# archinetai/audio-diffusion-pytorch

Measured on NVIDIA H100. Metric: audio-seconds/sec (2ch, 2^18 len) VSampler 50-step, higher is better.
Workload: dtype bf16

## Files before the change

### audio_diffusion_pytorch_b200/csrc/conv_gemm.cu

```cuda
#include "common.cuh"
#include "ptx.cuh"

namespace adp {

int g_debug[8] = {0, 0, 0, 0, 0, 0, 0, 0};

constexpr int kBM = 128;
constexpr int kMaxStages = 8;
constexpr int kMaxGroups = 8;
constexpr int kConsumers = 256;
constexpr int kGemmThreads = kConsumers + 32;
constexpr int kSmemPerSM = 228 * 1024;
constexpr int kSmemPerBlock = 227 * 1024;

struct Gemm2Params {
  __nv_bfloat16* out;
  const __nv_bfloat16* residual;
  const float* bias;
  const float* gate;
  double* stats;
  int B, T, tiles_per_batch, c_in, ldo;
  int n_pad, n_valid;
  int ntaps, tap_off0, up_factor;
  int groups, group_size, group_shift;
  int out_fp32, ld_gate;
  int n_tiles_n, total_tiles, tiles_per_cta;
  int a_rows;
  int kc;
  int k_stages;
  int n_stages;
  int a_sub_bytes, w_sub_bytes, stage_bytes, max_taps;
  int early_w;
  const double* gn_stats;
  const float* gn_gamma;
  const float* gn_beta;
  float gn_eps;
  int gn_groups;
};

struct TileInfo {
  int b, t0, n0, phase, ch0, ntaps, min_off;
};

__device__ __forceinline__ TileInfo tile_info(const Gemm2Params& p, int tile, int BN) {
  TileInfo ti;
  const int m_tile = tile / p.n_tiles_n;
  const int n_tile = tile - m_tile * p.n_tiles_n;
  ti.b = m_tile / p.tiles_per_batch;
  ti.t0 = (m_tile - ti.b * p.tiles_per_batch) * kBM;
  ti.n0 = n_tile * BN;
  ti.phase = ti.n0 / p.n_pad;
  ti.ch0 = ti.n0 - ti.phase * p.n_pad;
  if (p.up_factor > 1) {
    if (ti.phase == 0) { ti.ntaps = 2; ti.min_off = -1; }
    else if (ti.phase == p.up_factor - 1) { ti.ntaps = 2; ti.min_off = 0; }
    else { ti.ntaps = 1; ti.min_off = 0; }
  } else {
    ti.ntaps = p.ntaps;
    ti.min_off = p.tap_off0;
  }
  return ti;
}

__device__ __forceinline__ float silu_tanh(float z) {
  float t;
  asm("tanh.approx.f32 %0, %1;" : "=f"(t) : "f"(0.5f * z));
  const float hz = 0.5f * z;
  return fmaf(hz, t, hz);
}

struct WarpStats {
  int cur_g = -1;
  float s = 0.f, q = 0.f;
  __device__ __forceinline__ void flush(float (*slots)[8], int w, int lane) {
    const float ws = warp_sum(s), wq = warp_sum(q);
    if (lane == 0 && cur_g >= 0) { slots[2 * cur_g][w] += ws; slots[2 * cur_g + 1][w] += wq; }
    s = 0.f; q = 0.f;
  }
  __device__ __forceinline__ void add(float v, int g, float (*slots)[8], int w, int lane) {
    if (g != cur_g) { flush(slots, w, lane); cur_g = g; }
    s += v; q += v * v;
  }
};

struct NarrowStats {
  int ch0 = -1;
  float s[4] = {0.f, 0.f, 0.f, 0.f}, q[4] = {0.f, 0.f, 0.f, 0.f};
  __device__ __forceinline__ void add(int k, float v) { s[k] += v; q[k] += v * v; }
  __device__ __forceinline__ void flush(float (*slots)[8], int w, int lane, int shift, int groups) {
    if (ch0 >= 0) {
#pragma unroll
      for (int k = 0; k < 4; ++k) {
        float a = s[k], b = q[k];
#pragma unroll
        for (int o = 4; o < 32; o <<= 1) {
          a += __shfl_xor_sync(0xffffffffu, a, o);
          b += __shfl_xor_sync(0xffffffffu, b, o);
        }
        if (shift == 2) {
          a += __shfl_xor_sync(0xffffffffu, a, 1);
          b += __shfl_xor_sync(0xffffffffu, b, 1);
        }
        const int col = shift == 0 ? ch0 + 2 * lane + k : ch0 + 8 * k + 2 * (lane & 3);
        const int g = col >> shift;
        if (lane < 4 && (shift != 2 || !(lane & 1)) && (shift != 0 || k < 2) && g < groups) {
          slots[2 * g][w] += a;
          slots[2 * g + 1][w] += b;
        }
        s[k] = 0.f; q[k] = 0.f;
      }
    }
    ch0 = -1;
  }
};

template <int BN, int SW, bool XF, bool NARROW>
__global__ void __launch_bounds__(kGemmThreads, BN <= 32 ? 3 : (BN <= 64 ? 2 : 1))
conv_gemm2_kernel(const __grid_constant__ CUtensorMap tmA, const __grid_constant__ CUtensorMap tmW,
                  const Gemm2Params p) {
  static_assert(!NARROW || (BN <= 64 && !XF), "narrow statistics registers: BN <= 64 without XF");
  constexpr int BK = SW / 2;
  constexpr int NACC = BN / 2;
  constexpr uint32_t kWTapBytes = BN * SW;
  extern __shared__ uint8_t smem_raw[];
  __shared__ uint64_t full_bar[kMaxStages], empty_bar[kMaxStages];
  __shared__ float s_part[2 * kMaxGroups][8];
  __shared__ __align__(16) float s_coef[XF ? 2 * 1024 : 4];

  pdl_launch_dependents();
  const int warp = warp_id_uniform();
  const int lane = threadIdx.x & 31;
  const uint32_t raw = smem_u32(smem_raw);
  uint8_t* ring = smem_raw + ((1024u - (raw & 1023u)) & 1023u);

  const int tile_begin = blockIdx.x * p.tiles_per_cta;
  int tile_end = tile_begin + p.tiles_per_cta;
  if (tile_end > p.total_tiles) tile_end = p.total_tiles;

  if (threadIdx.x < 2 * kMaxGroups * 8) (&s_part[0][0])[threadIdx.x] = 0.f;
  if (warp == 8 && lane == 0) {
    for (int s = 0; s < p.n_stages; ++s) { mbar_init(&full_bar[s], 1); mbar_init(&empty_bar[s], 8); }
    fence_mbar_init();
    tma_prefetch_desc(&tmA);
    tma_prefetch_desc(&tmW);
  }
  __syncthreads();
  if (warp == 8) {
    const uint32_t a_bytes = static_cast<uint32_t>(p.a_rows) * SW;
    const int total_it = (tile_end - tile_begin) * p.k_stages;
    int early = 0;
    if (p.early_w) {
      early = total_it < p.n_stages ? total_it : p.n_stages;
      if (elect_one()) {
        int tile = tile_begin, ks = 0;
        for (int it = 0; it < early; ++it) {
          const TileInfo ti = tile_info(p, tile, BN);
          uint8_t* st = ring + it * p.stage_bytes;
          mbar_arrive_expect_tx(&full_bar[it], static_cast<uint32_t>(p.kc) * (a_bytes + ti.ntaps * kWTapBytes));
          for (int c = 0; c < p.kc; ++c) {
            const int k0 = (ks * p.kc + c) * BK;
            uint8_t* wdst = st + p.kc * p.a_sub_bytes + c * p.max_taps * p.w_sub_bytes;
            for (int tap = 0; tap < ti.ntaps; ++tap)
              tma_load_2d(wdst + tap * p.w_sub_bytes, &tmW, &full_bar[it], tap * p.c_in + k0, ti.n0);
          }
          if (++ks == p.k_stages) { ks = 0; ++tile; }
        }
      }
      __syncwarp();
    }
    pdl_wait();
    int s = 0, it = 0;
    uint32_t ph = 0;
    for (int tile = tile_begin; tile < tile_end; ++tile) {
      const TileInfo ti = tile_info(p, tile, BN);
      const uint32_t tx = static_cast<uint32_t>(p.kc) * (a_bytes + ti.ntaps * kWTapBytes);
      for (int ks = 0; ks < p.k_stages; ++ks, ++it) {
        const bool armed = it < early;
        if (!armed) mbar_wait(&empty_bar[s], ph ^ 1);
        uint8_t* st = ring + s * p.stage_bytes;
        if (elect_one()) {
          if (!armed) mbar_arrive_expect_tx(&full_bar[s], tx);
          for (int c = 0; c < p.kc; ++c) {
            const int k0 = (ks * p.kc + c) * BK;
            tma_load_3d(st + c * p.a_sub_bytes, &tmA, &full_bar[s], k0, ti.t0 + ti.min_off, ti.b);
            if (armed) continue;
            uint8_t* wdst = st + p.kc * p.a_sub_bytes + c * p.max_taps * p.w_sub_bytes;
            for (int tap = 0; tap < ti.ntaps; ++tap)
              tma_load_2d(wdst + tap * p.w_sub_bytes, &tmW, &full_bar[s], tap * p.c_in + k0, ti.n0);
          }
        }
        __syncwarp();
        if (++s == p.n_stages) { s = 0; ph ^= 1; }
      }
    }
    return;
  }

  pdl_wait();
  const int tid = threadIdx.x;
  const int wg = tid >> 7;
  const int r0 = wg * 64 + (warp & 3) * 16 + (lane >> 2);
  const int cq = 2 * (lane & 3);
  const bool do_stats = p.stats != nullptr;
  const bool narrow = NARROW && p.group_shift >= 0 && p.group_shift < 3;
  WarpStats acc_st;
  NarrowStats nar_st;
  int cur_b = -1, coef_b = -1;

  auto publish_stats = [&](int b_done) {
    acc_st.flush(s_part, warp, lane);
    acc_st.cur_g = -1;
    if (narrow) nar_st.flush(s_part, warp, lane, p.group_shift, p.groups);
    named_bar_sync(1, kConsumers);
    if (tid < 2 * p.groups) {
      float tot = 0.f;
#pragma unroll
      for (int w = 0; w < 8; ++w) { tot += s_part[tid][w]; s_part[tid][w] = 0.f; }
      if (tot != 0.f) atomicAdd(p.stats + static_cast<size_t>(b_done) * 2 * p.groups + tid, static_cast<double>(tot));
    }
    named_bar_sync(1, kConsumers);
  };

  const uint64_t desc0 = gmma_desc_kmajor<SW>(smem_u32(ring));
  const uint32_t stage_u = static_cast<uint32_t>(p.stage_bytes) >> 4;
  const uint32_t a_sub_u = static_cast<uint32_t>(p.a_sub_bytes) >> 4;
  const uint32_t w_sub_u = static_cast<uint32_t>(p.w_sub_bytes) >> 4;
  const uint32_t w_base_u = static_cast<uint32_t>(p.kc) * a_sub_u;
  const uint32_t wg_row_u = static_cast<uint32_t>(wg * 64 * SW) >> 4;
  int s = 0;
  uint32_t ph = 0;
  for (int tile = tile_begin; tile < tile_end; ++tile) {
    const TileInfo ti = tile_info(p, tile, BN);
    if constexpr (XF) {
      if (ti.b != coef_b) {
        named_bar_sync(1, kConsumers);
        const int gsz = p.c_in / p.gn_groups;
        const double inv_n = 1.0 / (static_cast<double>(gsz) * p.T);
        for (int ch = tid; ch < p.c_in; ch += kConsumers) {
          const int g = ch / gsz;
          const double mean = p.gn_stats[(static_cast<size_t>(ti.b) * p.gn_groups + g) * 2] * inv_n;
          const float var = fmaxf(static_cast<float>(
              p.gn_stats[(static_cast<size_t>(ti.b) * p.gn_groups + g) * 2 + 1] * inv_n - mean * mean), 0.f);
          const float ga = __ldg(p.gn_gamma + ch) * rsqrtf(var + p.gn_eps);
          s_coef[2 * ch] = ga;
          s_coef[2 * ch + 1] = __ldg(p.gn_beta + ch) - static_cast<float>(mean) * ga;
        }
        named_bar_sync(1, kConsumers);
        coef_b = ti.b;
      }
    }
    float acc[NACC];
    uint32_t accumulate = 0;
    int prev_s = -1;
    for (int ks = 0; ks < p.k_stages; ++ks) {
      mbar_wait(&full_bar[s], ph);
      if constexpr (XF) {
        constexpr int CPR = SW / 16;
        constexpr int CPT = CPR / 2 > 0 ? CPR / 2 : 1;
        uint8_t* st = ring + s * p.stage_bytes;
        for (int c = 0; c < p.kc; ++c) {
          uint8_t* sub = st + c * p.a_sub_bytes;
          const float* cf = s_coef + (ks * p.kc + c) * BK * 2;
          for (int rr = tid >> 1; rr < p.a_rows; rr += kConsumers / 2) {
            const int t = ti.t0 + ti.min_off + rr;
            if (t < 0 || t >= p.T) continue;
            const uint32_t row_off = static_cast<uint32_t>(rr) * SW;
            const int swz = (row_off >> 7) & (CPR - 1);
#pragma unroll
            for (int q = 0; q < CPT; ++q) {
              const int pc = (CPR >= 2) ? (tid & 1) * CPT + q : 0;
              if (CPR < 2 && (tid & 1)) continue;
              const int lc = pc ^ swz;
              uint4* ptr = reinterpret_cast<uint4*>(sub + row_off + pc * 16);
              const uint4 u = *ptr;
              const float4* c4 = reinterpret_cast<const float4*>(cf + lc * 16);
              const float4 k0 = c4[0], k1 = c4[1], k2 = c4[2], k3 = c4[3];
              const float2 f0 = unpack_bf16(u.x), f1 = unpack_bf16(u.y);
              const float2 f2 = unpack_bf16(u.z), f3 = unpack_bf16(u.w);
              uint4 o;
              o.x = pack_bf16(silu_tanh(f0.x * k0.x + k0.y), silu_tanh(f0.y * k0.z + k0.w));
              o.y = pack_bf16(silu_tanh(f1.x * k1.x + k1.y), silu_tanh(f1.y * k1.z + k1.w));
              o.z = pack_bf16(silu_tanh(f2.x * k2.x + k2.y), silu_tanh(f2.y * k2.z + k2.w));
              o.w = pack_bf16(silu_tanh(f3.x * k3.x + k3.y), silu_tanh(f3.y * k3.z + k3.w));
              *ptr = o;
            }
          }
        }
        fence_proxy_async_smem();
        named_bar_sync(1, kConsumers);
      }
      wgmma_fence();
      const uint64_t sdesc = desc0 + static_cast<uint64_t>(s * stage_u);
      for (int c = 0; c < p.kc; ++c) {
        const uint64_t adesc = sdesc + c * a_sub_u + wg_row_u;
        const uint64_t wdesc = sdesc + w_base_u + c * p.max_taps * w_sub_u;
        for (int tap = 0; tap < ti.ntaps; ++tap) {
#pragma unroll
          for (int kk = 0; kk < BK / 16; ++kk) {
            Wgmma<BN>::template ss<0, 0>(acc, adesc + ((tap * SW + kk * 32) >> 4),
                                         wdesc + tap * w_sub_u + ((kk * 32) >> 4), accumulate);
            accumulate = 1;
          }
        }
      }
      wgmma_commit();
      wgmma_wait<1>();
      if (prev_s >= 0) {
        __syncwarp();
        if (lane == 0) mbar_arrive(&empty_bar[prev_s]);
      }
      prev_s = s;
      if (++s == p.n_stages) { s = 0; ph ^= 1; }
    }
    wgmma_wait<0>();
    acc_fence(acc);
    __syncwarp();
    if (lane == 0) mbar_arrive(&empty_bar[prev_s]);

    if (do_stats && ti.b != cur_b) {
      if (cur_b >= 0) publish_stats(cur_b);
      cur_b = ti.b;
    }
    if (narrow && ti.ch0 != nar_st.ch0) {
      nar_st.flush(s_part, warp, lane, p.group_shift, p.groups);
      nar_st.ch0 = ti.ch0;
    }
    const int t_lo = ti.t0 + r0, t_hi = t_lo + 8;
    const bool ok_lo = t_lo < p.T, ok_hi = t_hi < p.T;
    const size_t col_off = static_cast<size_t>(ti.phase) * p.n_valid;
    const size_t off_lo = (static_cast<size_t>(ti.b) * p.T + (ok_lo ? t_lo : 0)) * p.ldo + col_off;
    const size_t off_hi = (static_cast<size_t>(ti.b) * p.T + (ok_hi ? t_hi : 0)) * p.ldo + col_off;
    const float* gate_row = p.gate ? p.gate + static_cast<size_t>(ti.b) * p.ld_gate : nullptr;
#pragma unroll
    for (int jb = 0; jb < BN / 8; ++jb) {
      if (ti.ch0 + jb * 8 >= p.n_valid) break;
      const int ch = ti.ch0 + jb * 8 + cq;
      const float2 bb = p.bias ? make_float2(__ldg(p.bias + ch), __ldg(p.bias + ch + 1)) : make_float2(0.f, 0.f);
      const float2 gg = gate_row ? make_float2(__ldg(gate_row + ch), __ldg(gate_row + ch + 1)) : make_float2(1.f, 1.f);
      float v[4];
      v[0] = (acc[4 * jb + 0] + bb.x) * gg.x; v[1] = (acc[4 * jb + 1] + bb.y) * gg.y;
      v[2] = (acc[4 * jb + 2] + bb.x) * gg.x; v[3] = (acc[4 * jb + 3] + bb.y) * gg.y;
      if (p.out_fp32) {
        float* o = reinterpret_cast<float*>(p.out);
        if (ok_lo) *reinterpret_cast<float2*>(o + off_lo + ch) = make_float2(v[0], v[1]);
        if (ok_hi) *reinterpret_cast<float2*>(o + off_hi + ch) = make_float2(v[2], v[3]);
        continue;
      }
      if (p.residual) {
        if (ok_lo) {
          const float2 r = unpack_bf16(__ldg(reinterpret_cast<const unsigned int*>(p.residual + off_lo + ch)));
          v[0] += r.x; v[1] += r.y;
        }
        if (ok_hi) {
          const float2 r = unpack_bf16(__ldg(reinterpret_cast<const unsigned int*>(p.residual + off_hi + ch)));
          v[2] += r.x; v[3] += r.y;
        }
      }
      const uint32_t o_lo = pack_bf16(v[0], v[1]), o_hi = pack_bf16(v[2], v[3]);
      if (ok_lo) *reinterpret_cast<uint32_t*>(p.out + off_lo + ch) = o_lo;
      if (ok_hi) *reinterpret_cast<uint32_t*>(p.out + off_hi + ch) = o_hi;
      if (do_stats) {
        const float2 q_lo = ok_lo ? unpack_bf16(o_lo) : make_float2(0.f, 0.f);
        const float2 q_hi = ok_hi ? unpack_bf16(o_hi) : make_float2(0.f, 0.f);
        if (p.group_shift >= 3) {
          const int g = (ti.ch0 + jb * 8) >> p.group_shift;
          acc_st.add(q_lo.x, g, s_part, warp, lane); acc_st.add(q_lo.y, g, s_part, warp, lane);
          acc_st.add(q_hi.x, g, s_part, warp, lane); acc_st.add(q_hi.y, g, s_part, warp, lane);
        } else if (narrow) {
          if (p.group_shift == 0) {
            nar_st.add(0, q_lo.x); nar_st.add(0, q_hi.x);
            nar_st.add(1, q_lo.y); nar_st.add(1, q_hi.y);
          } else if (jb < 4) {
            nar_st.add(jb, q_lo.x); nar_st.add(jb, q_lo.y);
            nar_st.add(jb, q_hi.x); nar_st.add(jb, q_hi.y);
          }
        } else {
          float cs[2] = {q_lo.x + q_hi.x, q_lo.y + q_hi.y};
          float cs2[2] = {q_lo.x * q_lo.x + q_hi.x * q_hi.x, q_lo.y * q_lo.y + q_hi.y * q_hi.y};
#pragma unroll
          for (int e = 0; e < 2; ++e)
#pragma unroll
            for (int o = 4; o < 32; o <<= 1) {
              cs[e] += __shfl_xor_sync(0xffffffffu, cs[e], o);
              cs2[e] += __shfl_xor_sync(0xffffffffu, cs2[e], o);
            }
#pragma unroll
          for (int i = 0; i < 8; ++i) {
            const float v = __shfl_sync(0xffffffffu, cs[i & 1], i >> 1);
            const float v2 = __shfl_sync(0xffffffffu, cs2[i & 1], i >> 1);
            const int g = (ti.ch0 + jb * 8 + i) / p.group_size;
            if (lane == 0) { s_part[2 * g][warp] += v; s_part[2 * g + 1][warp] += v2; }
          }
        }
      }
    }
  }
  if (do_stats && cur_b >= 0) publish_stats(cur_b);
}

template <int BN, int SW, bool XF, bool NARROW>
static int launch_gemm2(const adp_conv_gemm_args& a, cudaStream_t stream) {
  constexpr int BK = SW / 2;
  auto kernel = conv_gemm2_kernel<BN, SW, XF, NARROW>;
  const int tiles_per_batch = (a.T + kBM - 1) / kBM;
  const bool up = a.up_factor > 1;
  const int max_taps = up ? 2 : a.ntaps;
  const int span = up ? 1 : a.ntaps - 1;
  const int a_rows = kBM + span;
  const int k_chunks = a.c_in / BK;

  Gemm2Params p;
  p.a_sub_bytes = (a_rows * SW + 1023) / 1024 * 1024;
  p.w_sub_bytes = (BN * SW + 1023) / 1024 * 1024;
  p.max_taps = max_taps;
  const int chunk_bytes = p.a_sub_bytes + max_taps * p.w_sub_bytes;

  const int w_iters = k_chunks * max_taps;
  int occ = 1;
  if (BN <= 64 && w_iters <= 8) occ = 3;
  else if (BN <= 128 && w_iters <= 12) occ = 2;
  if (XF && occ > (BN <= 64 ? 2 : 1)) occ = BN <= 64 ? 2 : 1;
  if (g_debug[3] > 0) occ = g_debug[3];
  static int static_smem = -1;
  if (static_smem < 0) {
    cudaFuncAttributes fa;
    ADP_CUDA(cudaFuncGetAttributes(&fa, kernel));
    static_smem = static_cast<int>(fa.sharedSizeBytes);
  }
  auto budget_of = [&](int o) {
    int per_cta = kSmemPerSM / o - 1024;
    if (per_cta > kSmemPerBlock) per_cta = kSmemPerBlock;
    return per_cta - static_smem - 1024;
  };
  while (occ > 1 && budget_of(occ) < 2 * chunk_bytes) --occ;
  const int budget = budget_of(occ);
  int kc = 1;
  while (kc * 2 <= 4 && k_chunks % (kc * 2) == 0 && kc * max_taps * (BK / 16) < 8 &&
         2 * (kc * 2) * chunk_bytes <= budget)
    kc *= 2;
  if (g_debug[5] > 0 && k_chunks % g_debug[5] == 0) kc = g_debug[5];
  p.kc = kc;
  p.k_stages = k_chunks / kc;
  p.stage_bytes = kc * chunk_bytes;
  int n_stages = budget / p.stage_bytes;
  if (n_stages > kMaxStages) n_stages = kMaxStages;
  if (n_stages < 2)
    return set_error("adp_conv_gemm: stage of %d bytes does not fit (BN=%d)", p.stage_bytes, BN);
  p.n_stages = n_stages;
  const size_t smem = static_cast<size_t>(n_stages) * p.stage_bytes + 1024;

  CUtensorMap tmA, tmW;
  {
    const uint64_t dims[3] = {(uint64_t)a.c_in, (uint64_t)a.T, (uint64_t)a.B};
    const uint64_t strides[2] = {(uint64_t)a.lda * 2, (uint64_t)a.T * a.lda * 2};
    const uint32_t box[3] = {(uint32_t)BK, (uint32_t)a_rows, 1};
    if (int e = make_tmap_bf16(&tmA, a.a, 3, dims, strides, box, SW)) return e;
  }
  {
    const uint64_t dims[2] = {(uint64_t)a.k_total, (uint64_t)a.phases * a.n_pad};
    const uint64_t strides[1] = {(uint64_t)a.k_total * 2};
    const uint32_t box[2] = {(uint32_t)BK, (uint32_t)BN};
    if (int e = make_tmap_bf16(&tmW, a.w, 2, dims, strides, box, SW)) return e;
  }

  static SmemAttrCache smem_cache;
  ADP_CUDA(ensure_dyn_smem(kernel, smem, smem_cache));
  int occ_hw = 1;
  if (cudaOccupancyMaxActiveBlocksPerMultiprocessor(&occ_hw, kernel, kGemmThreads, smem) != cudaSuccess ||
      occ_hw < 1)
    occ_hw = 1;
  if (occ > occ_hw) occ = occ_hw;

  p.out = static_cast<__nv_bfloat16*>(a.out);
  p.residual = static_cast<const __nv_bfloat16*>(a.residual);
  p.bias = a.bias;
  p.gate = a.gate;
  p.stats = a.stats;
  p.B = a.B;
  p.T = a.T;
  p.tiles_per_batch = tiles_per_batch;
  p.c_in = a.c_in;
  p.ldo = a.ldo;
  p.n_pad = a.n_pad;
  p.n_valid = a.n_valid;
  p.ntaps = a.ntaps;
  p.tap_off0 = a.tap_off[0];
  p.up_factor = a.up_factor;
  p.groups = a.stats ? a.groups : 0;
  p.group_size = a.stats ? a.n_valid / a.groups : 1;
  p.group_shift = -1;
  for (int sft = 0; sft < 16; ++sft)
    if ((1 << sft) == p.group_size) p.group_shift = sft;
  p.out_fp32 = a.out_fp32;
  p.ld_gate = a.ld_gate > 0 ? a.ld_gate : a.n_valid;
  p.n_tiles_n = a.phases * a.n_pad / BN;
  p.total_tiles = a.B * tiles_per_batch * p.n_tiles_n;
  p.a_rows = a_rows;
  p.early_w = g_debug[2];
  p.gn_stats = a.gn_stats;
  p.gn_gamma = a.gn_gamma;
  p.gn_beta = a.gn_beta;
  p.gn_eps = a.gn_eps;
  p.gn_groups = a.gn_groups > 0 ? a.gn_groups : 1;

  const int slots = occ * num_sms();
  int grid = p.total_tiles < slots ? p.total_tiles : slots;
  p.tiles_per_cta = (p.total_tiles + grid - 1) / grid;
  grid = (p.total_tiles + p.tiles_per_cta - 1) / p.tiles_per_cta;
  ADP_CUDA(launch_k(kernel, dim3(grid), dim3(kGemmThreads), smem, stream, tmA, tmW, p));
  ADP_LAUNCH_CHECK();
  return 0;
}

template <int SW>
static int dispatch_bn2(const adp_conv_gemm_args& a, int bn, cudaStream_t s) {
  if (a.gn_stats) {
    switch (bn) {
      case 16: return launch_gemm2<16, SW, true, false>(a, s);
      case 32: return launch_gemm2<32, SW, true, false>(a, s);
      case 64: return launch_gemm2<64, SW, true, false>(a, s);
      case 128: return launch_gemm2<128, SW, true, false>(a, s);
      case 256: return launch_gemm2<256, SW, true, false>(a, s);
    }
  }
  const int group_size = a.stats ? a.n_valid / a.groups : 0;
  const bool narrow = group_size == 1 || group_size == 2 || group_size == 4 || g_debug[7] != 0;
  switch (bn) {
    case 16: return narrow ? launch_gemm2<16, SW, false, true>(a, s) : launch_gemm2<16, SW, false, false>(a, s);
    case 32: return narrow ? launch_gemm2<32, SW, false, true>(a, s) : launch_gemm2<32, SW, false, false>(a, s);
    case 64: return narrow ? launch_gemm2<64, SW, false, true>(a, s) : launch_gemm2<64, SW, false, false>(a, s);
    case 128: return launch_gemm2<128, SW, false, false>(a, s);
    case 256: return launch_gemm2<256, SW, false, false>(a, s);
  }
  return set_error("adp_conv_gemm: unsupported N tile %d", bn);
}

}

namespace adp { extern int g_mid_threads; }

extern "C" int adp_debug_set(int key, int value) {
  if (key == 8) {
    if (value != 128 && value != 256) return adp::set_error("adp_debug_set: key 8 takes 128 or 256");
    adp::g_mid_threads = value;
    return 0;
  }
  if (key < 0 || key >= 8) return adp::set_error("adp_debug_set: bad key %d", key);
  adp::g_debug[key] = value;
  if (key == 6) adp::g_pdl = value;
  return 0;
}

extern "C" int adp_conv_gemm(const adp_conv_gemm_args* args, adp_stream_t stream) {
  using namespace adp;
  ADP_CHECK(args != nullptr, "adp_conv_gemm: null args");
  const adp_conv_gemm_args& a = *args;
  ADP_CHECK(a.a && a.w && a.out, "adp_conv_gemm: null a/w/out");
  ADP_CHECK(a.B > 0 && a.T > 0, "adp_conv_gemm: bad B=%d T=%d", a.B, a.T);
  ADP_CHECK(a.c_in >= 16 && a.c_in % 16 == 0, "adp_conv_gemm: c_in=%d must be a multiple of 16",
            a.c_in);
  ADP_CHECK(a.lda % 8 == 0 && a.ldo % 8 == 0 && a.k_total % 8 == 0 && a.lda >= a.c_in,
            "adp_conv_gemm: pitches lda=%d ldo=%d k_total=%d must be multiples of 8", a.lda, a.ldo,
            a.k_total);
  ADP_CHECK(a.n_valid > 0 && a.n_valid % 8 == 0 && a.n_valid <= a.n_pad && a.n_pad % 16 == 0,
            "adp_conv_gemm: n_valid=%d n_pad=%d", a.n_valid, a.n_pad);
  ADP_CHECK(a.phases >= 1, "adp_conv_gemm: phases=%d", a.phases);
  ADP_CHECK(a.ld_gate % 4 == 0, "adp_conv_gemm: ld_gate=%d must be a multiple of 4", a.ld_gate);
  if (a.up_factor > 1) {
    ADP_CHECK(a.phases == a.up_factor, "adp_conv_gemm: phases (%d) != up_factor (%d)", a.phases,
              a.up_factor);
    ADP_CHECK(a.k_total >= 2 * a.c_in, "adp_conv_gemm: upsample weights need 2 tap slots");
  } else {
    ADP_CHECK(a.ntaps >= 1 && a.ntaps <= 3 && a.phases == 1, "adp_conv_gemm: ntaps=%d phases=%d",
              a.ntaps, a.phases);
    ADP_CHECK(a.k_total >= a.ntaps * a.c_in, "adp_conv_gemm: k_total too small");
    for (int i = 1; i < a.ntaps; ++i)
      ADP_CHECK(a.tap_off[i] == a.tap_off[i - 1] + 1,
                "adp_conv_gemm: tap offsets must be consecutive and ascending");
  }
  if (a.out_fp32) {
    ADP_CHECK(!a.residual && !a.stats, "adp_conv_gemm: out_fp32 excludes residual/stats");
  }
  if (a.gn_stats) {
    ADP_CHECK(a.c_in <= 1024, "adp_conv_gemm: fused GroupNorm supports c_in <= 1024");
    ADP_CHECK(a.gn_gamma && a.gn_beta && a.gn_groups > 0 && a.c_in % a.gn_groups == 0 && a.lda == a.c_in,
              "adp_conv_gemm: fused GroupNorm needs gamma/beta, groups | c_in and a dense input");
  }
  if (a.stats) {
    ADP_CHECK(a.groups > 0 && a.groups <= kMaxGroups && a.n_valid % a.groups == 0,
              "adp_conv_gemm: groups=%d n_valid=%d (fused statistics handle <= %d groups)",
              a.groups, a.n_valid, kMaxGroups);
  }
  int bn = a.block_n;
  if (bn == 0) {
    const long m_tiles = (long)a.B * ((a.T + kBM - 1) / kBM);
    const int k_per_tile = (a.up_factor > 1 ? 2 : a.ntaps) * a.c_in;
    const int widest = !a.gn_stats && k_per_tile <= 1024 ? 64 : 128;
    bn = 16;
    for (int cand = widest; cand >= 16; cand >>= 1) {
      if (a.n_pad % cand) continue;
      const long tiles = m_tiles * (a.phases * a.n_pad / cand);
      if (tiles >= 96 || cand <= 64) { bn = cand; break; }
    }
  }
  ADP_CHECK(a.n_pad % bn == 0, "adp_conv_gemm: N tile %d does not divide n_pad %d", bn, a.n_pad);
  cudaStream_t s = as_stream(stream);
  if (a.c_in % 64 == 0) return dispatch_bn2<128>(a, bn, s);
  if (a.c_in % 32 == 0) return dispatch_bn2<64>(a, bn, s);
  return dispatch_bn2<32>(a, bn, s);
}
```

### audio_diffusion_pytorch_b200/csrc/ptx.cuh

```cuda
#pragma once
#include <cuda.h>
#include <cuda_bf16.h>
#include <cuda_runtime.h>
#include <stdint.h>

namespace adp {

__device__ __forceinline__ uint32_t smem_u32(const void* p) {
  return static_cast<uint32_t>(__cvta_generic_to_shared(p));
}

__device__ __forceinline__ int warp_id_uniform() {
  return __shfl_sync(0xffffffffu, static_cast<int>(threadIdx.x >> 5), 0);
}
__device__ __forceinline__ bool elect_one() {
  uint32_t pred;
  asm volatile(
      "{\n\t.reg .pred p;\n\t"
      "elect.sync _|p, 0xffffffff;\n\t"
      "selp.u32 %0, 1, 0, p;\n\t}"
      : "=r"(pred));
  return pred != 0;
}

__device__ __forceinline__ void mbar_init(uint64_t* bar, uint32_t count) {
  asm volatile("mbarrier.init.shared::cta.b64 [%0], %1;" ::"r"(smem_u32(bar)), "r"(count));
}
__device__ __forceinline__ void fence_mbar_init() {
  asm volatile("fence.mbarrier_init.release.cluster;" ::: "memory");
}
__device__ __forceinline__ void fence_proxy_async_smem() {
  asm volatile("fence.proxy.async.shared::cta;" ::: "memory");
}
__device__ __forceinline__ void mbar_arrive_expect_tx(uint64_t* bar, uint32_t bytes) {
  asm volatile("mbarrier.arrive.expect_tx.shared::cta.b64 _, [%0], %1;" ::"r"(smem_u32(bar)),
               "r"(bytes)
               : "memory");
}
__device__ __forceinline__ void mbar_arrive(uint64_t* bar) {
  asm volatile("mbarrier.arrive.shared::cta.b64 _, [%0];" ::"r"(smem_u32(bar)) : "memory");
}
__device__ __forceinline__ bool mbar_try_wait(uint64_t* bar, uint32_t parity) {
  uint32_t ok;
  asm volatile(
      "{\n\t.reg .pred p;\n\t"
      "mbarrier.try_wait.parity.shared::cta.b64 p, [%1], %2;\n\t"
      "selp.u32 %0, 1, 0, p;\n\t}"
      : "=r"(ok)
      : "r"(smem_u32(bar)), "r"(parity)
      : "memory");
  return ok != 0;
}
static __device__ __noinline__ void mbar_wait_slow(uint64_t* bar, uint32_t parity) {
  uint32_t spins = 0;
  while (!mbar_try_wait(bar, parity)) {
    if (++spins > (1u << 24)) __trap();
  }
}
__device__ __forceinline__ void mbar_wait(uint64_t* bar, uint32_t parity) {
  if (mbar_try_wait(bar, parity)) return;
  mbar_wait_slow(bar, parity);
}

__device__ __forceinline__ void tma_prefetch_desc(const CUtensorMap* m) {
  asm volatile("prefetch.tensormap [%0];" ::"l"(reinterpret_cast<uint64_t>(m)) : "memory");
}
__device__ __forceinline__ void tma_load_2d(void* smem_dst, const CUtensorMap* m, uint64_t* bar,
                                            int c0, int c1) {
  asm volatile(
      "cp.async.bulk.tensor.2d.shared::cluster.global.mbarrier::complete_tx::bytes"
      " [%0], [%1, {%3, %4}], [%2];" ::"r"(smem_u32(smem_dst)),
      "l"(reinterpret_cast<uint64_t>(m)), "r"(smem_u32(bar)), "r"(c0), "r"(c1)
      : "memory");
}
__device__ __forceinline__ void tma_load_3d(void* smem_dst, const CUtensorMap* m, uint64_t* bar,
                                            int c0, int c1, int c2) {
  asm volatile(
      "cp.async.bulk.tensor.3d.shared::cluster.global.mbarrier::complete_tx::bytes"
      " [%0], [%1, {%3, %4, %5}], [%2];" ::"r"(smem_u32(smem_dst)),
      "l"(reinterpret_cast<uint64_t>(m)), "r"(smem_u32(bar)), "r"(c0), "r"(c1), "r"(c2)
      : "memory");
}
__device__ __forceinline__ void tma_load_4d(void* smem_dst, const CUtensorMap* m, uint64_t* bar,
                                            int c0, int c1, int c2, int c3) {
  asm volatile(
      "cp.async.bulk.tensor.4d.shared::cluster.global.mbarrier::complete_tx::bytes"
      " [%0], [%1, {%3, %4, %5, %6}], [%2];" ::"r"(smem_u32(smem_dst)),
      "l"(reinterpret_cast<uint64_t>(m)), "r"(smem_u32(bar)), "r"(c0), "r"(c1), "r"(c2), "r"(c3)
      : "memory");
}

__device__ __forceinline__ void wgmma_fence() {
  asm volatile("wgmma.fence.sync.aligned;" ::: "memory");
}
__device__ __forceinline__ void wgmma_commit() {
  asm volatile("wgmma.commit_group.sync.aligned;" ::: "memory");
}
template <int N>
__device__ __forceinline__ void wgmma_wait() {
  asm volatile("wgmma.wait_group.sync.aligned %0;" ::"n"(N) : "memory");
}
template <int R>
__device__ __forceinline__ void acc_fence(float (&d)[R]) {
#pragma unroll
  for (int i = 0; i < R; ++i) asm volatile("" : "+f"(d[i])::"memory");
}

template <int N> struct Wgmma;
template <> struct Wgmma<16> {
  template <int TA, int TB>
  static __device__ __forceinline__ void ss(float (&d)[8], uint64_t a, uint64_t b, uint32_t acc) {
    asm volatile(
        "{\n\t.reg .pred p;\n\tsetp.ne.b32 p, %10, 0;\n\t"
        "wgmma.mma_async.sync.aligned.m64n16k16.f32.bf16.bf16 {%0, %1, %2, %3, %4, %5, %6, %7}, %8, %9, p, 1, 1, %11, %12;\n\t}"
        : "+f"(d[0]), "+f"(d[1]), "+f"(d[2]), "+f"(d[3]), "+f"(d[4]), "+f"(d[5]), "+f"(d[6]), "+f"(d[7])
        : "l"(a), "l"(b), "r"(acc), "n"(TA), "n"(TB));
  }
};
template <> struct Wgmma<32> {
  template <int TA, int TB>
  static __device__ __forceinline__ void ss(float (&d)[16], uint64_t a, uint64_t b, uint32_t acc) {
    asm volatile(
        "{\n\t.reg .pred p;\n\tsetp.ne.b32 p, %18, 0;\n\t"
        "wgmma.mma_async.sync.aligned.m64n32k16.f32.bf16.bf16 {%0, %1, %2, %3, %4, %5, %6, %7, %8, %9, %10, %11, %12, %13, %14, %15}, %16, %17, p, 1, 1, %19, %20;\n\t}"
        : "+f"(d[0]), "+f"(d[1]), "+f"(d[2]), "+f"(d[3]), "+f"(d[4]), "+f"(d[5]), "+f"(d[6]), "+f"(d[7]), "+f"(d[8]), "+f"(d[9]), "+f"(d[10]), "+f"(d[11]), "+f"(d[12]), "+f"(d[13]), "+f"(d[14]), "+f"(d[15])
        : "l"(a), "l"(b), "r"(acc), "n"(TA), "n"(TB));
  }
  template <int TB>
  static __device__ __forceinline__ void rs(float (&d)[16], const uint32_t (&a)[4], uint64_t b, uint32_t acc) {
    asm volatile(
        "{\n\t.reg .pred p;\n\tsetp.ne.b32 p, %21, 0;\n\t"
        "wgmma.mma_async.sync.aligned.m64n32k16.f32.bf16.bf16 {%0, %1, %2, %3, %4, %5, %6, %7, %8, %9, %10, %11, %12, %13, %14, %15}, {%16, %17, %18, %19}, %20, p, 1, 1, %22;\n\t}"
        : "+f"(d[0]), "+f"(d[1]), "+f"(d[2]), "+f"(d[3]), "+f"(d[4]), "+f"(d[5]), "+f"(d[6]), "+f"(d[7]), "+f"(d[8]), "+f"(d[9]), "+f"(d[10]), "+f"(d[11]), "+f"(d[12]), "+f"(d[13]), "+f"(d[14]), "+f"(d[15])
        : "r"(a[0]), "r"(a[1]), "r"(a[2]), "r"(a[3]), "l"(b), "r"(acc), "n"(TB));
  }
};
template <> struct Wgmma<64> {
  template <int TA, int TB>
  static __device__ __forceinline__ void ss(float (&d)[32], uint64_t a, uint64_t b, uint32_t acc) {
    asm volatile(
        "{\n\t.reg .pred p;\n\tsetp.ne.b32 p, %34, 0;\n\t"
        "wgmma.mma_async.sync.aligned.m64n64k16.f32.bf16.bf16 {%0, %1, %2, %3, %4, %5, %6, %7, %8, %9, %10, %11, %12, %13, %14, %15, %16, %17, %18, %19, %20, %21, %22, %23, %24, %25, %26, %27, %28, %29, %30, %31}, %32, %33, p, 1, 1, %35, %36;\n\t}"
        : "+f"(d[0]), "+f"(d[1]), "+f"(d[2]), "+f"(d[3]), "+f"(d[4]), "+f"(d[5]), "+f"(d[6]), "+f"(d[7]), "+f"(d[8]), "+f"(d[9]), "+f"(d[10]), "+f"(d[11]), "+f"(d[12]), "+f"(d[13]), "+f"(d[14]), "+f"(d[15]), "+f"(d[16]), "+f"(d[17]), "+f"(d[18]), "+f"(d[19]), "+f"(d[20]), "+f"(d[21]), "+f"(d[22]), "+f"(d[23]), "+f"(d[24]), "+f"(d[25]), "+f"(d[26]), "+f"(d[27]), "+f"(d[28]), "+f"(d[29]), "+f"(d[30]), "+f"(d[31])
        : "l"(a), "l"(b), "r"(acc), "n"(TA), "n"(TB));
  }
  template <int TB>
  static __device__ __forceinline__ void rs(float (&d)[32], const uint32_t (&a)[4], uint64_t b, uint32_t acc) {
    asm volatile(
        "{\n\t.reg .pred p;\n\tsetp.ne.b32 p, %37, 0;\n\t"
        "wgmma.mma_async.sync.aligned.m64n64k16.f32.bf16.bf16 {%0, %1, %2, %3, %4, %5, %6, %7, %8, %9, %10, %11, %12, %13, %14, %15, %16, %17, %18, %19, %20, %21, %22, %23, %24, %25, %26, %27, %28, %29, %30, %31}, {%32, %33, %34, %35}, %36, p, 1, 1, %38;\n\t}"
        : "+f"(d[0]), "+f"(d[1]), "+f"(d[2]), "+f"(d[3]), "+f"(d[4]), "+f"(d[5]), "+f"(d[6]), "+f"(d[7]), "+f"(d[8]), "+f"(d[9]), "+f"(d[10]), "+f"(d[11]), "+f"(d[12]), "+f"(d[13]), "+f"(d[14]), "+f"(d[15]), "+f"(d[16]), "+f"(d[17]), "+f"(d[18]), "+f"(d[19]), "+f"(d[20]), "+f"(d[21]), "+f"(d[22]), "+f"(d[23]), "+f"(d[24]), "+f"(d[25]), "+f"(d[26]), "+f"(d[27]), "+f"(d[28]), "+f"(d[29]), "+f"(d[30]), "+f"(d[31])
        : "r"(a[0]), "r"(a[1]), "r"(a[2]), "r"(a[3]), "l"(b), "r"(acc), "n"(TB));
  }
};
template <> struct Wgmma<128> {
  template <int TA, int TB>
  static __device__ __forceinline__ void ss(float (&d)[64], uint64_t a, uint64_t b, uint32_t acc) {
    asm volatile(
        "{\n\t.reg .pred p;\n\tsetp.ne.b32 p, %66, 0;\n\t"
        "wgmma.mma_async.sync.aligned.m64n128k16.f32.bf16.bf16 {%0, %1, %2, %3, %4, %5, %6, %7, %8, %9, %10, %11, %12, %13, %14, %15, %16, %17, %18, %19, %20, %21, %22, %23, %24, %25, %26, %27, %28, %29, %30, %31, %32, %33, %34, %35, %36, %37, %38, %39, %40, %41, %42, %43, %44, %45, %46, %47, %48, %49, %50, %51, %52, %53, %54, %55, %56, %57, %58, %59, %60, %61, %62, %63}, %64, %65, p, 1, 1, %67, %68;\n\t}"
        : "+f"(d[0]), "+f"(d[1]), "+f"(d[2]), "+f"(d[3]), "+f"(d[4]), "+f"(d[5]), "+f"(d[6]), "+f"(d[7]), "+f"(d[8]), "+f"(d[9]), "+f"(d[10]), "+f"(d[11]), "+f"(d[12]), "+f"(d[13]), "+f"(d[14]), "+f"(d[15]), "+f"(d[16]), "+f"(d[17]), "+f"(d[18]), "+f"(d[19]), "+f"(d[20]), "+f"(d[21]), "+f"(d[22]), "+f"(d[23]), "+f"(d[24]), "+f"(d[25]), "+f"(d[26]), "+f"(d[27]), "+f"(d[28]), "+f"(d[29]), "+f"(d[30]), "+f"(d[31]), "+f"(d[32]), "+f"(d[33]), "+f"(d[34]), "+f"(d[35]), "+f"(d[36]), "+f"(d[37]), "+f"(d[38]), "+f"(d[39]), "+f"(d[40]), "+f"(d[41]), "+f"(d[42]), "+f"(d[43]), "+f"(d[44]), "+f"(d[45]), "+f"(d[46]), "+f"(d[47]), "+f"(d[48]), "+f"(d[49]), "+f"(d[50]), "+f"(d[51]), "+f"(d[52]), "+f"(d[53]), "+f"(d[54]), "+f"(d[55]), "+f"(d[56]), "+f"(d[57]), "+f"(d[58]), "+f"(d[59]), "+f"(d[60]), "+f"(d[61]), "+f"(d[62]), "+f"(d[63])
        : "l"(a), "l"(b), "r"(acc), "n"(TA), "n"(TB));
  }
  template <int TB>
  static __device__ __forceinline__ void rs(float (&d)[64], const uint32_t (&a)[4], uint64_t b, uint32_t acc) {
    asm volatile(
        "{\n\t.reg .pred p;\n\tsetp.ne.b32 p, %69, 0;\n\t"
        "wgmma.mma_async.sync.aligned.m64n128k16.f32.bf16.bf16 {%0, %1, %2, %3, %4, %5, %6, %7, %8, %9, %10, %11, %12, %13, %14, %15, %16, %17, %18, %19, %20, %21, %22, %23, %24, %25, %26, %27, %28, %29, %30, %31, %32, %33, %34, %35, %36, %37, %38, %39, %40, %41, %42, %43, %44, %45, %46, %47, %48, %49, %50, %51, %52, %53, %54, %55, %56, %57, %58, %59, %60, %61, %62, %63}, {%64, %65, %66, %67}, %68, p, 1, 1, %70;\n\t}"
        : "+f"(d[0]), "+f"(d[1]), "+f"(d[2]), "+f"(d[3]), "+f"(d[4]), "+f"(d[5]), "+f"(d[6]), "+f"(d[7]), "+f"(d[8]), "+f"(d[9]), "+f"(d[10]), "+f"(d[11]), "+f"(d[12]), "+f"(d[13]), "+f"(d[14]), "+f"(d[15]), "+f"(d[16]), "+f"(d[17]), "+f"(d[18]), "+f"(d[19]), "+f"(d[20]), "+f"(d[21]), "+f"(d[22]), "+f"(d[23]), "+f"(d[24]), "+f"(d[25]), "+f"(d[26]), "+f"(d[27]), "+f"(d[28]), "+f"(d[29]), "+f"(d[30]), "+f"(d[31]), "+f"(d[32]), "+f"(d[33]), "+f"(d[34]), "+f"(d[35]), "+f"(d[36]), "+f"(d[37]), "+f"(d[38]), "+f"(d[39]), "+f"(d[40]), "+f"(d[41]), "+f"(d[42]), "+f"(d[43]), "+f"(d[44]), "+f"(d[45]), "+f"(d[46]), "+f"(d[47]), "+f"(d[48]), "+f"(d[49]), "+f"(d[50]), "+f"(d[51]), "+f"(d[52]), "+f"(d[53]), "+f"(d[54]), "+f"(d[55]), "+f"(d[56]), "+f"(d[57]), "+f"(d[58]), "+f"(d[59]), "+f"(d[60]), "+f"(d[61]), "+f"(d[62]), "+f"(d[63])
        : "r"(a[0]), "r"(a[1]), "r"(a[2]), "r"(a[3]), "l"(b), "r"(acc), "n"(TB));
  }
};
// ... 116 lines not shown
```

Before: 168.3.

## Stage conv GEMM epilogue through shared memory with TMA residual load and store

For BN<=64 non-fp32 GEMMs, the producer warp now prefetches the residual tile into a swizzled shared-memory slot via TMA. Consumers apply bias, gate and residual there, write bf16 output back into the slot, and one thread issues a TMA tensor store. This replaces scattered 4-byte global loads and stores with bulk transfers and overlaps the residual fetch with the main loop. The cost is extra shared memory, which can reduce pipeline stages or occupancy (a fallback to the unstaged kernel exists), plus a named barrier per tile and a serialized wait on store completion. Occupancy for 1-tap, deep-K cases is also lowered from 3 to 2.

```diff
diff --git a/audio_diffusion_pytorch_b200/csrc/conv_gemm.cu b/audio_diffusion_pytorch_b200/csrc/conv_gemm.cu
--- a/audio_diffusion_pytorch_b200/csrc/conv_gemm.cu
+++ b/audio_diffusion_pytorch_b200/csrc/conv_gemm.cu
@@ -30,6 +30,7 @@
   int k_stages;
   int n_stages;
   int a_sub_bytes, w_sub_bytes, stage_bytes, max_taps;
+  int n_slots, slot_bytes, slot_base;
   int early_w;
   const double* gn_stats;
   const float* gn_gamma;
@@ -114,16 +115,20 @@
   }
 };
 
-template <int BN, int SW, bool XF, bool NARROW>
+template <int BN, int SW, bool XF, bool NARROW, bool STAGED>
 __global__ void __launch_bounds__(kGemmThreads, BN <= 32 ? 3 : (BN <= 64 ? 2 : 1))
 conv_gemm2_kernel(const __grid_constant__ CUtensorMap tmA, const __grid_constant__ CUtensorMap tmW,
+                  const __grid_constant__ CUtensorMap tmO, const __grid_constant__ CUtensorMap tmR,
                   const Gemm2Params p) {
   static_assert(!NARROW || (BN <= 64 && !XF), "narrow statistics registers: BN <= 64 without XF");
+  static_assert(!STAGED || (BN <= 64 && !XF), "staged epilogue: BN <= 64 without XF");
   constexpr int BK = SW / 2;
   constexpr int NACC = BN / 2;
   constexpr uint32_t kWTapBytes = BN * SW;
+  constexpr uint32_t kSlotRow = BN * 2;
   extern __shared__ uint8_t smem_raw[];
   __shared__ uint64_t full_bar[kMaxStages], empty_bar[kMaxStages];
+  __shared__ uint64_t slot_full[STAGED ? kMaxStages : 1], slot_empty[STAGED ? kMaxStages : 1];
   __shared__ float s_part[2 * kMaxGroups][8];
   __shared__ __align__(16) float s_coef[XF ? 2 * 1024 : 4];
 
@@ -140,9 +145,15 @@
   if (threadIdx.x < 2 * kMaxGroups * 8) (&s_part[0][0])[threadIdx.x] = 0.f;
   if (warp == 8 && lane == 0) {
     for (int s = 0; s < p.n_stages; ++s) { mbar_init(&full_bar[s], 1); mbar_init(&empty_bar[s], 8); }
+    if constexpr (STAGED)
+      for (int s = 0; s < p.n_slots; ++s) { mbar_init(&slot_full[s], 1); mbar_init(&slot_empty[s], 1); }
     fence_mbar_init();
     tma_prefetch_desc(&tmA);
     tma_prefetch_desc(&tmW);
+    if constexpr (STAGED) {
+      tma_prefetch_desc(&tmO);
+      if (p.residual) tma_prefetch_desc(&tmR);
+    }
   }
   __syncthreads();
   if (warp == 8) {
@@ -169,8 +180,8 @@
       __syncwarp();
     }
     pdl_wait();
-    int s = 0, it = 0;
-    uint32_t ph = 0;
+    int s = 0, it = 0, sl = 0;
+    uint32_t ph = 0, sph = 0;
     for (int tile = tile_begin; tile < tile_end; ++tile) {
       const TileInfo ti = tile_info(p, tile, BN);
       const uint32_t tx = static_cast<uint32_t>(p.kc) * (a_bytes + ti.ntaps * kWTapBytes);
@@ -192,6 +203,20 @@
         __syncwarp();
         if (++s == p.n_stages) { s = 0; ph ^= 1; }
       }
+      if constexpr (STAGED) {
+        mbar_wait(&slot_empty[sl], sph ^ 1);
+        if (elect_one()) {
+          uint8_t* slot = ring + p.slot_base + sl * p.slot_bytes;
+          if (p.residual) {
+            mbar_arrive_expect_tx(&slot_full[sl], kBM * kSlotRow);
+            tma_load_4d(slot, &tmR, &slot_full[sl], ti.ch0, ti.phase, ti.t0, ti.b);
+          } else {
+            mbar_arrive(&slot_full[sl]);
+          }
+        }
+        __syncwarp();
+        if (++sl == p.n_slots) { sl = 0; sph ^= 1; }
+      }
     }
     return;
   }
@@ -227,8 +252,8 @@
   const uint32_t w_sub_u = static_cast<uint32_t>(p.w_sub_bytes) >> 4;
   const uint32_t w_base_u = static_cast<uint32_t>(p.kc) * a_sub_u;
   const uint32_t wg_row_u = static_cast<uint32_t>(wg * 64 * SW) >> 4;
-  int s = 0;
-  uint32_t ph = 0;
+  int s = 0, sl = 0;
+  uint32_t ph = 0, sph = 0;
   for (int tile = tile_begin; tile < tile_end; ++tile) {
     const TileInfo ti = tile_info(p, tile, BN);
     if constexpr (XF) {
@@ -331,6 +356,10 @@
     const size_t off_lo = (static_cast<size_t>(ti.b) * p.T + (ok_lo ? t_lo : 0)) * p.ldo + col_off;
     const size_t off_hi = (static_cast<size_t>(ti.b) * p.T + (ok_hi ? t_hi : 0)) * p.ldo + col_off;
     const float* gate_row = p.gate ? p.gate + static_cast<size_t>(ti.b) * p.ld_gate : nullptr;
+    uint8_t* slot = ring + p.slot_base + sl * p.slot_bytes;
+    const uint32_t srow_lo = static_cast<uint32_t>(r0) * kSlotRow, srow_hi = srow_lo + 8 * kSlotRow;
+    const uint32_t swz_lo = (srow_lo >> 7) & (BN / 8 - 1), swz_hi = (srow_hi >> 7) & (BN / 8 - 1);
+    if constexpr (STAGED) mbar_wait(&slot_full[sl], sph);
 #pragma unroll
     for (int jb = 0; jb < BN / 8; ++jb) {
       if (ti.ch0 + jb * 8 >= p.n_valid) break;
@@ -340,25 +369,41 @@
       float v[4];
       v[0] = (acc[4 * jb + 0] + bb.x) * gg.x; v[1] = (acc[4 * jb + 1] + bb.y) * gg.y;
       v[2] = (acc[4 * jb + 2] + bb.x) * gg.x; v[3] = (acc[4 * jb + 3] + bb.y) * gg.y;
-      if (p.out_fp32) {
-        float* o = reinterpret_cast<float*>(p.out);
-        if (ok_lo) *reinterpret_cast<float2*>(o + off_lo + ch) = make_float2(v[0], v[1]);
-        if (ok_hi) *reinterpret_cast<float2*>(o + off_hi + ch) = make_float2(v[2], v[3]);
-        continue;
-      }
-      if (p.residual) {
-        if (ok_lo) {
-          const float2 r = unpack_bf16(__ldg(reinterpret_cast<const unsigned int*>(p.residual + off_lo + ch)));
-          v[0] += r.x; v[1] += r.y;
-        }
-        if (ok_hi) {
-          const float2 r = unpack_bf16(__ldg(reinterpret_cast<const unsigned int*>(p.residual + off_hi + ch)));
-          v[2] += r.x; v[3] += r.y;
-        }
-      }
-      const uint32_t o_lo = pack_bf16(v[0], v[1]), o_hi = pack_bf16(v[2], v[3]);
-      if (ok_lo) *reinterpret_cast<uint32_t*>(p.out + off_lo + ch) = o_lo;
-      if (ok_hi) *reinterpret_cast<uint32_t*>(p.out + off_hi + ch) = o_hi;
+      uint32_t o_lo, o_hi;
+      if constexpr (STAGED) {
+        uint32_t* s_lo = reinterpret_cast<uint32_t*>(slot + srow_lo + ((jb ^ swz_lo) << 4) + 2 * cq);
+        uint32_t* s_hi = reinterpret_cast<uint32_t*>(slot + srow_hi + ((jb ^ swz_hi) << 4) + 2 * cq);
+        if (p.residual) {
+          const float2 r_lo = unpack_bf16(*s_lo), r_hi = unpack_bf16(*s_hi);
+          v[0] += r_lo.x; v[1] += r_lo.y;
+          v[2] += r_hi.x; v[3] += r_hi.y;
+        }
+        o_lo = pack_bf16(v[0], v[1]);
+        o_hi = pack_bf16(v[2], v[3]);
+        *s_lo = o_lo;
+        *s_hi = o_hi;
+      } else {
+        if (p.out_fp32) {
+          float* o = reinterpret_cast<float*>(p.out);
+          if (ok_lo) *reinterpret_cast<float2*>(o + off_lo + ch) = make_float2(v[0], v[1]);
+          if (ok_hi) *reinterpret_cast<float2*>(o + off_hi + ch) = make_float2(v[2], v[3]);
+          continue;
+        }
+        if (p.residual) {
+          if (ok_lo) {
+            const float2 r = unpack_bf16(__ldg(reinterpret_cast<const unsigned int*>(p.residual + off_lo + ch)));
+            v[0] += r.x; v[1] += r.y;
+          }
+          if (ok_hi) {
+            const float2 r = unpack_bf16(__ldg(reinterpret_cast<const unsigned int*>(p.residual + off_hi + ch)));
+            v[2] += r.x; v[3] += r.y;
+          }
+        }
+        o_lo = pack_bf16(v[0], v[1]);
+        o_hi = pack_bf16(v[2], v[3]);
+        if (ok_lo) *reinterpret_cast<uint32_t*>(p.out + off_lo + ch) = o_lo;
+        if (ok_hi) *reinterpret_cast<uint32_t*>(p.out + off_hi + ch) = o_hi;
+      }
       if (do_stats) {
         const float2 q_lo = ok_lo ? unpack_bf16(o_lo) : make_float2(0.f, 0.f);
         const float2 q_hi = ok_hi ? unpack_bf16(o_hi) : make_float2(0.f, 0.f);
@@ -394,14 +439,25 @@
         }
       }
     }
+    if constexpr (STAGED) {
+      fence_proxy_async_smem();
+      named_bar_sync(1, kConsumers);
+      if (tid == 0) {
+        tma_store_4d(&tmO, slot, ti.ch0, ti.phase, ti.t0, ti.b);
+        bulk_commit_group();
+        bulk_wait_group_read<0>();
+        mbar_arrive(&slot_empty[sl]);
+      }
+      if (++sl == p.n_slots) { sl = 0; sph ^= 1; }
+    }
   }
   if (do_stats && cur_b >= 0) publish_stats(cur_b);
 }
 
-template <int BN, int SW, bool XF, bool NARROW>
+template <int BN, int SW, bool XF, bool NARROW, bool STAGED>
 static int launch_gemm2(const adp_conv_gemm_args& a, cudaStream_t stream) {
   constexpr int BK = SW / 2;
-  auto kernel = conv_gemm2_kernel<BN, SW, XF, NARROW>;
+  auto kernel = conv_gemm2_kernel<BN, SW, XF, NARROW, STAGED>;
   const int tiles_per_batch = (a.T + kBM - 1) / kBM;
   const bool up = a.up_factor > 1;
   const int max_taps = up ? 2 : a.ntaps;
@@ -417,10 +473,11 @@
 
   const int w_iters = k_chunks * max_taps;
   int occ = 1;
-  if (BN <= 64 && w_iters <= 8) occ = 3;
+  if (BN <= 64 && w_iters <= 8) occ = max_taps == 1 && k_chunks >= 4 ? 2 : 3;
   else if (BN <= 128 && w_iters <= 12) occ = 2;
   if (XF && occ > (BN <= 64 ? 2 : 1)) occ = BN <= 64 ? 2 : 1;
   if (g_debug[3] > 0) occ = g_debug[3];
+  const int occ_req = occ;
   static int static_smem = -1;
   if (static_smem < 0) {
     cudaFuncAttributes fa;
@@ -432,22 +489,46 @@
     if (per_cta > kSmemPerBlock) per_cta = kSmemPerBlock;
     return per_cta - static_smem - 1024;
   };
-  while (occ > 1 && budget_of(occ) < 2 * chunk_bytes) --occ;
+  const int slot_bytes = STAGED ? (kBM * BN * 2 + 1023) / 1024 * 1024 : 0;
+  while (occ > 1 && budget_of(occ) < 2 * chunk_bytes + slot_bytes) --occ;
   const int budget = budget_of(occ);
   int kc = 1;
   while (kc * 2 <= 4 && k_chunks % (kc * 2) == 0 && kc * max_taps * (BK / 16) < 8 &&
-         2 * (kc * 2) * chunk_bytes <= budget)
+         2 * (kc * 2) * chunk_bytes + slot_bytes <= budget)
     kc *= 2;
   if (g_debug[5] > 0 && k_chunks % g_debug[5] == 0) kc = g_debug[5];
   p.kc = kc;
   p.k_stages = k_chunks / kc;
   p.stage_bytes = kc * chunk_bytes;
-  int n_stages = budget / p.stage_bytes;
+  int n_stages = budget / p.stage_bytes, n_slots = 0;
   if (n_stages > kMaxStages) n_stages = kMaxStages;
+  if (STAGED) {
+    for (; n_stages >= 2; --n_stages) {
+      n_slots = (n_stages + p.k_stages - 1) / p.k_stages;
+      while (n_slots > 1 && n_stages * p.stage_bytes + n_slots * slot_bytes > budget) --n_slots;
+      if (n_stages * p.stage_bytes + n_slots * slot_bytes <= budget) break;
+    }
+  }
+  if (STAGED && p.k_stages >= 4) {
+    int occ_d = occ_req;
+    while (occ_d > 1 && budget_of(occ_d) < 2 * chunk_bytes) --occ_d;
+    const int budget_d = budget_of(occ_d);
+    int kc_d = 1;
+    while (kc_d * 2 <= 4 && k_chunks % (kc_d * 2) == 0 && kc_d * max_taps * (BK / 16) < 8 &&
+           2 * (kc_d * 2) * chunk_bytes <= budget_d)
+      kc_d *= 2;
+    if (g_debug[5] > 0 && k_chunks % g_debug[5] == 0) kc_d = g_debug[5];
+    int n_d = budget_d / (kc_d * chunk_bytes);
+    if (n_d > kMaxStages) n_d = kMaxStages;
+    if (n_stages < n_d) return launch_gemm2<BN, SW, XF, NARROW, false>(a, stream);
+  }
   if (n_stages < 2)
     return set_error("adp_conv_gemm: stage of %d bytes does not fit (BN=%d)", p.stage_bytes, BN);
   p.n_stages = n_stages;
-  const size_t smem = static_cast<size_t>(n_stages) * p.stage_bytes + 1024;
+  p.n_slots = n_slots;
+  p.slot_bytes = slot_bytes;
+  p.slot_base = n_stages * p.stage_bytes;
+  const size_t smem = static_cast<size_t>(n_stages) * p.stage_bytes + n_slots * slot_bytes + 1024;
 
   CUtensorMap tmA, tmW;
   {
@@ -461,6 +542,17 @@
     const uint64_t strides[1] = {(uint64_t)a.k_total * 2};
     const uint32_t box[2] = {(uint32_t)BK, (uint32_t)BN};
     if (int e = make_tmap_bf16(&tmW, a.w, 2, dims, strides, box, SW)) return e;
+  }
+  CUtensorMap tmO, tmR;
+  memset(&tmO, 0, sizeof(tmO));
+  memset(&tmR, 0, sizeof(tmR));
+  if (STAGED) {
+    const uint64_t dims[4] = {(uint64_t)a.n_valid, (uint64_t)a.phases, (uint64_t)a.T, (uint64_t)a.B};
+    const uint64_t strides[3] = {(uint64_t)a.n_valid * 2, (uint64_t)a.ldo * 2, (uint64_t)a.T * a.ldo * 2};
+    const uint32_t box[4] = {(uint32_t)BN, 1, (uint32_t)kBM, 1};
+    if (int e = make_tmap_bf16(&tmO, a.out, 4, dims, strides, box, BN * 2)) return e;
+    if (a.residual)
+      if (int e = make_tmap_bf16(&tmR, a.residual, 4, dims, strides, box, BN * 2)) return e;
   }
 
   static SmemAttrCache smem_cache;
@@ -507,30 +599,39 @@
   int grid = p.total_tiles < slots ? p.total_tiles : slots;
   p.tiles_per_cta = (p.total_tiles + grid - 1) / grid;
   grid = (p.total_tiles + p.tiles_per_cta - 1) / p.tiles_per_cta;
-  ADP_CUDA(launch_k(kernel, dim3(grid), dim3(kGemmThreads), smem, stream, tmA, tmW, p));
+  ADP_CUDA(launch_k(kernel, dim3(grid), dim3(kGemmThreads), smem, stream, tmA, tmW, tmO, tmR, p));
   ADP_LAUNCH_CHECK();
   return 0;
+}
+
+template <int BN, int SW>
+static int dispatch_staged(const adp_conv_gemm_args& a, bool narrow, bool staged, cudaStream_t s) {
+  if (staged) return narrow ? launch_gemm2<BN, SW, false, true, true>(a, s) : launch_gemm2<BN, SW, false, false, true>(a, s);
+  return narrow ? launch_gemm2<BN, SW, false, true, false>(a, s) : launch_gemm2<BN, SW, false, false, false>(a, s);
 }
 
 template <int SW>
 static int dispatch_bn2(const adp_conv_gemm_args& a, int bn, cudaStream_t s) {
   if (a.gn_stats) {
     switch (bn) {
-      case 16: return launch_gemm2<16, SW, true, false>(a, s);
-      case 32: return launch_gemm2<32, SW, true, false>(a, s);
-      case 64: return launch_gemm2<64, SW, true, false>(a, s);
-      case 128: return launch_gemm2<128, SW, true, false>(a, s);
-      case 256: return launch_gemm2<256, SW, true, false>(a, s);
+      case 16: return launch_gemm2<16, SW, true, false, false>(a, s);
+      case 32: return launch_gemm2<32, SW, true, false, false>(a, s);
+      case 64: return launch_gemm2<64, SW, true, false, false>(a, s);
+      case 128: return launch_gemm2<128, SW, true, false, false>(a, s);
+      case 256: return launch_gemm2<256, SW, true, false, false>(a, s);
     }
   }
   const int group_size = a.stats ? a.n_valid / a.groups : 0;
   const bool narrow = group_size == 1 || group_size == 2 || group_size == 4 || g_debug[7] != 0;
+  const bool staged = !a.out_fp32 && a.n_valid >= bn && g_debug[4] == 0 &&
+                      (reinterpret_cast<uintptr_t>(a.out) & 15) == 0 &&
+                      (reinterpret_cast<uintptr_t>(a.residual) & 15) == 0;
   switch (bn) {
-    case 16: return narrow ? launch_gemm2<16, SW, false, true>(a, s) : launch_gemm2<16, SW, false, false>(a, s);
-    case 32: return narrow ? launch_gemm2<32, SW, false, true>(a, s) : launch_gemm2<32, SW, false, false>(a, s);
-    case 64: return narrow ? launch_gemm2<64, SW, false, true>(a, s) : launch_gemm2<64, SW, false, false>(a, s);
-    case 128: return launch_gemm2<128, SW, false, false>(a, s);
-    case 256: return launch_gemm2<256, SW, false, false>(a, s);
+    case 16: return dispatch_staged<16, SW>(a, narrow, staged, s);
+    case 32: return dispatch_staged<32, SW>(a, narrow, staged, s);
+    case 64: return dispatch_staged<64, SW>(a, narrow, staged, s);
+    case 128: return launch_gemm2<128, SW, false, false, false>(a, s);
+    case 256: return launch_gemm2<256, SW, false, false, false>(a, s);
   }
   return set_error("adp_conv_gemm: unsupported N tile %d", bn);
 }
diff --git a/audio_diffusion_pytorch_b200/csrc/ptx.cuh b/audio_diffusion_pytorch_b200/csrc/ptx.cuh
--- a/audio_diffusion_pytorch_b200/csrc/ptx.cuh
+++ b/audio_diffusion_pytorch_b200/csrc/ptx.cuh
@@ -88,6 +88,21 @@
       " [%0], [%1, {%3, %4, %5, %6}], [%2];" ::"r"(smem_u32(smem_dst)),
       "l"(reinterpret_cast<uint64_t>(m)), "r"(smem_u32(bar)), "r"(c0), "r"(c1), "r"(c2), "r"(c3)
       : "memory");
+}
+__device__ __forceinline__ void tma_store_4d(const CUtensorMap* m, const void* smem_src, int c0,
+                                             int c1, int c2, int c3) {
+  asm volatile(
+      "cp.async.bulk.tensor.4d.global.shared::cta.bulk_group [%0, {%2, %3, %4, %5}], [%1];" ::"l"(
+          reinterpret_cast<uint64_t>(m)),
+      "r"(smem_u32(smem_src)), "r"(c0), "r"(c1), "r"(c2), "r"(c3)
+      : "memory");
+}
+__device__ __forceinline__ void bulk_commit_group() {
+  asm volatile("cp.async.bulk.commit_group;" ::: "memory");
+}
+template <int N>
+__device__ __forceinline__ void bulk_wait_group_read() {
+  asm volatile("cp.async.bulk.wait_group.read %0;" ::"n"(N) : "memory");
 }
 
 __device__ __forceinline__ void wgmma_fence() {
```

After: 179.4, median of 6. 1.07x the previous value.
